# zhaodong-liu/GRAM

Hardware: AMD Instinct MI355X
Metric: users/sec @ beam=20 top-20 gen, Beauty T5-base; Recall@5 parity (higher is better)
Workload: dtype f16x3

## Files before the change

gram_amd/_lib.py:

```python
from __future__ import annotations

import ctypes as C
import os

_HERE = os.path.dirname(os.path.abspath(__file__))
LIB_PATH = os.environ.get("GRAM_LIB") or os.path.join(_HERE, "csrc", "libgram_hip.so")

GRAM_MAX_BEAMS = 64
GRAM_MAX_DEC_LEN = 64
GRAM_MAX_PASSAGE_LEN = 128
GRAM_MAX_LONG_PASSAGE_LEN = 512
GRAM_MAX_FUSED_LEN = 4096
GRAM_MAX_LONG_FUSED_LEN = 16384
GRAM_KEY_BITS_LONG_WORDS, GRAM_KEY_BITS_LONG_STRIDE = 512, 528
EPI_BF16, EPI_BF16_RELU, EPI_F32_ADD, EPI_F32, EPI_KV_BANK = range(5)
K_GEMM, K_ENC_ATTN, K_CROSS_ATTN, K_DEC_SELF_ATTN, K_ROWOPS, K_LSE, K_BEAM = range(7)
E_ARG, E_WORKSPACE, E_BEAM, E_NONFINITE = -1, -2, -3, -4
ABI_VERSION = 7
GRAM_TAIL_ENTRY_ROWS = 64
GRAM_TAIL_MAX_STEPS = 16
GRAM_MAX_USER_ITEMS = 4096
ITEMS_EXCLUDE, ITEMS_ALLOW = 0, 1
MAX_PIECES = 2
SPLIT_NPROD = (0, 1, 3)
# ... 136 lines not shown
    "gram_workspace_encoder_x_offset": (i64, [vp, C.c_int, C.c_int, C.c_int, C.c_int, C.c_int]),
    "gram_encode_fused": (C.c_int, [vp, vp, vp, C.c_int, C.c_int, C.c_int, vp, i64, C.c_int, C.c_int, vp, vp]),
    "gram_decode_step": (C.c_int, [vp, vp, vp, vp, C.c_int, C.c_int, C.c_int, C.c_int, C.c_int, C.c_int, vp, i64, vp, vp]),
    "gram_prof_pp_clock": (C.c_int, [C.POINTER(C.c_double), C.c_int]),
    "gram_prof_pp_clock_enable": (C.c_int, [C.c_int]),
    "gram_debug_set_gemm_variant": (C.c_int, [C.c_int]),
    "gram_gemm_stream_max_m": (C.c_int, []),
    "gram_debug_set_live_rows": (C.c_int, [C.c_int]),
    "gram_debug_set_token_tables": (C.c_int, [C.c_int]),
    "gram_debug_set_beam_chunked": (C.c_int, [C.c_int]),
    "gram_debug_set_beam_chunk_capacity": (C.c_int, [C.c_int]),
    "gram_debug_set_stage_pieces": (C.c_int, [C.POINTER(i32), C.c_int]),
    "gram_debug_stream_read": (C.c_int, [vp, C.c_size_t, vp, vp]),
    "gram_debug_stream_read_variant": (C.c_int, [vp, C.c_size_t, vp, C.c_int, C.c_int, vp]),
    "gram_prof_enable": (C.c_int, [C.c_uint32, C.c_int]),
    "gram_prof_reset": (C.c_int, []),
    "gram_prof_collect": (C.c_int, [C.c_int, C.POINTER(C.c_double), C.POINTER(i64), C.POINTER(C.c_double), C.POINTER(i64)]),
    "gram_rmsnorm_bf16_map": (C.c_int, [vp, vp, vp, C.c_int, C.c_int, f32, f32, vp, C.c_int, C.c_int, vp, vp]),
    "gram_generate_ex": (C.c_int, [vp, vp, vp, C.c_int, C.c_int, C.c_int, C.c_int, C.c_int, C.c_int, f32, C.POINTER(Trie),
                                   C.POINTER(Compaction), vp, i64, vp, vp, C.POINTER(i32), vp]),
    "gram_user_items_prepare": (C.c_int, [vp, C.c_int, vp, C.c_int, C.c_int, vp, vp, C.c_int, vp]),
    "gram_beam_step_sparse_items": (C.c_int, [C.POINTER(BeamState), C.POINTER(Trie), vp, vp, C.c_int, vp, C.c_int, C.c_int, C.c_int, vp,
                                              C.POINTER(UserItems), vp]),
    "gram_beam_step_sparse_split_items": (C.c_int, [C.POINTER(BeamState), C.POINTER(Trie), vp, vp, C.c_int, vp, C.c_int, C.c_int, C.c_int,
                                                    vp, C.c_int, C.POINTER(UserItems), vp]),
    "gram_greedy_step_items": (C.c_int, [C.POINTER(BeamState), C.POINTER(Trie), vp, C.c_int, C.c_int, C.POINTER(UserItems), vp]),
    "gram_generate_items": (C.c_int, [vp, vp, vp, C.c_int, C.c_int, C.c_int, C.c_int, C.c_int, C.c_int, f32, C.POINTER(Trie),
                                      C.POINTER(Compaction), C.POINTER(UserItems), vp, i64, vp, vp, C.POINTER(i32), vp]),
    "gram_encode_passages": (C.c_int, [vp, vp, vp, C.c_int, C.c_int, vp, i64, vp, vp]),
    "gram_gather_passage_x": (C.c_int, [vp, vp, vp, C.c_int, C.c_int, C.c_int, C.c_int, vp]),
    "gram_live_rows": (C.c_int, [C.POINTER(BeamState), C.POINTER(Trie), C.POINTER(LiveRows), vp]),
    "gram_dec_self_attn_live": (C.c_int, [vp, vp, vp, vp, vp, vp, C.c_int, C.c_int, vp, C.c_int, C.c_int, C.c_int, vp]),
    "gram_cross_attn_decode_live": (C.c_int, [vp, vp, vp, vp, vp, C.c_int, vp, vp, C.c_int, C.c_int, C.c_int, vp]),
    "gram_beam_step_sparse_live": (C.c_int, [C.POINTER(BeamState), C.POINTER(Trie), vp, vp, C.c_int, vp, C.c_int, C.c_int, vp, vp]),
    "gram_gemm_bf16_split": (C.c_int, [vp, vp, vp, C.c_int, C.c_int, C.c_int, C.c_int, C.c_int, C.c_int, C.POINTER(KVBank),
                                       C.POINTER(NormFusion), C.POINTER(Split), vp]),
    "gram_gemm_bf16_lse_split": (C.c_int, [vp, vp, vp, vp, C.c_int, C.c_int, C.c_int, C.c_int, C.c_int, C.POINTER(Split), vp]),
    "gram_embed_ex_split": (C.c_int, [vp, vp, C.c_int, vp, vp, vp, C.c_int, C.c_int, C.c_int, C.c_int, vp]),
    "gram_rmsnorm_bf16_split": (C.c_int, [vp, vp, vp, C.c_int, C.c_int, f32, f32, vp, C.c_int, C.c_int, vp, C.c_int, vp]),
    "gram_enc_self_attn_split": (C.c_int, [vp, vp, vp, vp, C.c_int, C.c_int, C.c_int, C.c_int, i64, vp]),
    "gram_cross_attn_decode_split": (C.c_int, [vp, vp, vp, vp, vp, C.c_int, C.c_int, C.c_int, C.c_int, vp, vp, C.c_int, i64, i64, vp, vp]),
    "gram_enc_self_attn_rows_split": (C.c_int, [vp, vp, vp, vp, vp, C.c_int, C.c_int, C.c_int, C.c_int, i64, vp]),
    "gram_enc_self_attn_long_split": (C.c_int, [vp, vp, vp, vp, C.c_int, C.c_int, C.c_int, C.c_int, i64, vp]),
    "gram_enc_self_attn_long_rows_split": (C.c_int, [vp, vp, vp, vp, vp, C.c_int, C.c_int, C.c_int, C.c_int, i64, vp]),
    "gram_model_set_max_passage_len": (C.c_int, [vp, C.c_int]),
    "gram_mask_key_bits": (C.c_int, [vp, vp, C.c_int, C.c_int, vp]),
    "gram_model_set_max_fused_len": (C.c_int, [vp, C.c_int]),
    "gram_mask_key_bits_long": (C.c_int, [vp, vp, C.c_int, C.c_int, vp]),
    "gram_cross_attn_long_scratch_bytes": (i64, [C.c_int, C.c_int, C.c_int]),
    "gram_cross_attn_long_split": (C.c_int, [vp, vp, vp, vp, vp, C.c_int, C.c_int, C.c_int, C.c_int, vp, vp, C.c_int, i64, i64, vp, vp, vp]),
    "gram_cross_attn_rows_long_split": (C.c_int, [vp, vp, vp, vp, vp, C.c_int, C.c_int, C.c_int, C.c_int, C.c_int, i64, i64, vp, vp, vp, vp]),
    "gram_dec_self_attn_split": (C.c_int, [vp, vp, vp, vp, vp, vp, C.c_int, C.c_int, vp, C.c_int, C.c_int, C.c_int, C.c_int, i64, i64, vp]),
    "gram_dec_self_attn_rows_split": (C.c_int, [vp, vp, vp, vp, vp, vp, vp, C.c_int, C.c_int, vp, C.c_int, C.c_int, C.c_int, C.c_int, i64, i64,
                                                vp]),
    "gram_beam_step_sparse_split": (C.c_int, [C.POINTER(BeamState), C.POINTER(Trie), vp, vp, C.c_int, vp, C.c_int, C.c_int, C.c_int,
                                              vp, C.c_int, vp]),
    "gram_generate": (C.c_int, [vp, vp, vp, C.c_int, C.c_int, C.c_int, C.c_int, C.c_int, C.c_int, f32, C.POINTER(Trie),
                                vp, i64, vp, vp, C.POINTER(i32), vp]),
    "gram_workspace_bytes_tf": (i64, [vp, C.c_int, C.c_int, C.c_int, C.c_int, C.c_int]),
    "gram_teacher_forced": (C.c_int, [vp, vp, vp, C.c_int, C.c_int, C.c_int, C.POINTER(Compaction), vp, vp, C.c_int, C.c_int, vp, i64,
                                      vp, vp, vp, vp]),
    "gram_dec_self_attn_tf_split": (C.c_int, [vp, vp, vp, C.c_int, C.c_int, C.c_int, C.c_int, i64, vp]),
    "gram_cross_attn_rows_split": (C.c_int, [vp, vp, vp, vp, vp, C.c_int, C.c_int, C.c_int, C.c_int, C.c_int, i64, i64, vp, vp, vp]),
    "gram_label_logprob_split": (C.c_int, [vp, vp, vp, C.c_int, vp, vp, C.c_int, C.c_int, C.c_int, C.c_int, vp, vp, vp]),
    "gram_cross_attn_probs_split": (C.c_int, [vp, vp, vp, vp, C.c_int, C.c_int, C.c_int, C.c_int, C.c_int, i64, i64, vp, vp]),
    "gram_xattn_head_sum": (C.c_int, [vp, vp, C.c_int, C.c_int, C.c_int, C.c_int, C.c_int, vp]),
    "gram_xattn_passage_scores": (C.c_int, [vp, vp, vp, C.c_int, C.c_int, C.c_int, C.c_int, f32, vp]),
    "gram_teacher_forced_ex": (C.c_int, [vp, vp, vp, C.c_int, C.c_int, C.c_int, C.POINTER(Compaction), vp, vp, C.c_int, C.c_int, vp, i64,
                                         vp, vp, vp, C.POINTER(XattnOut), vp]),
    "gram_cross_attn_token_scores_split": (C.c_int, [vp, vp, vp, C.c_int, C.c_int, C.c_int, C.c_int, C.c_int, i64, i64, vp, C.c_int, vp]),
    "gram_teacher_forced_scores": (C.c_int, [vp, vp, vp, C.c_int, C.c_int, C.c_int, C.POINTER(Compaction), vp, vp, C.c_int, C.c_int, vp,
                                             i64, vp, vp, vp, C.POINTER(XattnScores), vp]),
    "gram_dec_self_attn_tree_split": (C.c_int, [vp, vp, vp, vp, vp, C.c_int, C.c_int, C.c_int, C.c_int, C.c_int, i64, vp]),
    "gram_trie_repeat_tokens": (C.c_int, [vp, vp, C.c_int, C.c_int, vp]),
    "gram_trie_leaf_logprob_split": (C.c_int, [vp, vp, vp, C.c_int, vp, C.POINTER(TrieRows), C.c_int, C.c_int, C.c_int, vp, vp, vp, vp]),
    "gram_workspace_bytes_trie": (i64, [vp, C.c_int, C.c_int, C.c_int, C.c_int]),
    "gram_score_trie": (C.c_int, [vp, vp, vp, C.c_int, C.c_int, C.c_int, C.POINTER(Compaction), C.POINTER(Trie), C.POINTER(TrieRows), vp,
                                  i64, vp, vp, vp]),
    "gram_tail_forest": (C.c_int, [C.POINTER(BeamState), C.POINTER(Trie), C.POINTER(TrieTail), C.POINTER(Forest), C.c_int, vp]),
    "gram_tail_rowpos": (C.c_int, [C.POINTER(BeamState), C.POINTER(Trie), C.POINTER(Forest), vp]),
    "gram_scatter_rows": (C.c_int, [vp, vp, vp, C.c_int, C.c_int, C.c_int, vp]),
    "gram_cross_attn_entries_split": (C.c_int, [vp, vp, vp, vp, vp, C.c_int, C.c_int, C.c_int, C.c_int, vp, vp, C.c_int, i64, i64, vp,
                                                vp]),
    "gram_workspace_bytes_tail": (i64, [vp, C.c_int, C.c_int, C.c_int, C.c_int, C.c_int, C.c_int]),
    "gram_generate_tail": (C.c_int, [vp, vp, vp, C.c_int, C.c_int, C.c_int, C.c_int, C.c_int, C.c_int, f32, C.POINTER(Trie),
                                     C.POINTER(Compaction), C.POINTER(TrieTail), vp, i64, vp, vp, C.POINTER(i32), vp]),
    "gram_debug_set_tail_pass": (C.c_int, [C.c_int]),
    "gram_tail_pass_wanted": (C.c_int, [vp, C.c_int, C.c_int, C.c_int]),
    "gram_debug_set_tail_capacity": (C.c_int, [C.c_int]),
    "gram_debug_set_tail_level_capacity": (C.c_int, [C.c_int]),
    "gram_debug_tail_last": (C.c_int, [C.POINTER(i32)]),
    "gram_debug_workspace_beam_state": (C.c_int, [vp, vp, C.c_int, C.c_int, C.c_int, C.c_int, C.c_int, C.POINTER(BeamState)]),
    "gram_sample_step": (C.c_int, [C.POINTER(BeamState), C.POINTER(Trie), vp, vp, vp, C.c_int, vp, C.c_int, C.c_int, C.c_int, C.c_int,
                                   C.POINTER(SampleParams), vp, C.c_int, vp, vp, vp]),
    "gram_sample_step_items": (C.c_int, [C.POINTER(BeamState), C.POINTER(Trie), vp, vp, vp, C.c_int, vp, C.c_int, C.c_int, C.c_int, C.c_int,
                                         C.POINTER(SampleParams), vp, C.c_int, vp, vp, C.POINTER(UserItems), vp]),
    "gram_sample_finalize": (C.c_int, [C.POINTER(BeamState), C.c_int, vp, vp, vp, vp, vp, vp, vp]),
    "gram_sample_capacity": (C.c_int, []),
    "gram_debug_set_sample_capacity": (C.c_int, [C.c_int]),
    "gram_workspace_bytes_sample": (i64, [vp, C.c_int, C.c_int, C.c_int, C.c_int, C.c_int, C.c_int]),
    "gram_sample": (C.c_int, [vp, vp, vp, C.c_int, C.c_int, C.c_int, C.c_int, C.c_int, C.POINTER(Trie), C.POINTER(Compaction),
                              C.POINTER(SampleParams), vp, vp, i64, vp, vp, vp, C.POINTER(i32), vp]),
    "gram_sample_items": (C.c_int, [vp, vp, vp, C.c_int, C.c_int, C.c_int, C.c_int, C.c_int, C.POINTER(Trie), C.POINTER(Compaction),
                                    C.POINTER(UserItems), C.POINTER(SampleParams), vp, vp, i64, vp, vp, vp, C.POINTER(i32), vp]),
}

for _old, _new in (("gram_gemm_bf16", "gram_gemm_f16"), ("gram_gemm_bf16_ex", "gram_gemm_f16_ex"), ("gram_gemm_bf16_split", "gram_gemm_f16_split"),
                   ("gram_gemm_bf16_lse", "gram_gemm_f16_lse"), ("gram_gemm_bf16_lse_split", "gram_gemm_f16_lse_split"),
                   ("gram_rmsnorm_bf16", "gram_rmsnorm_f16"), ("gram_rmsnorm_bf16_map", "gram_rmsnorm_f16_map"),
                   ("gram_rmsnorm_bf16_split", "gram_rmsnorm_f16_split")):
    SIGNATURES[_new] = SIGNATURES[_old]

_lib = None


def load() -> C.CDLL:
    global _lib
    if _lib is not None:
        return _lib
    import torch
    if not os.path.exists(LIB_PATH):
        raise ImportError(
            f"{LIB_PATH} not found: the HIP extension is not built (run __graft_entry__.build() or "
            "`make -C gram_amd/csrc`).  gram_amd has no CPU fallback."
        )
    lib = C.CDLL(LIB_PATH)
    for name, (res, args) in SIGNATURES.items():
        fn = getattr(lib, name)
        fn.restype = res
        fn.argtypes = args
    if lib.gram_abi_version() != ABI_VERSION:
        raise ImportError("libgram_hip.so ABI version mismatch")
    _lib = lib
    return lib


class GramHipError(RuntimeError):
    pass


def piece_dtype():
    import torch
    return torch.float16 if load().gram_piece_format() == 1 else torch.bfloat16


def check(code: int, what: str) -> None:
    if code == 0:
        return
    names = {E_ARG: "GRAM_E_ARG (bad shape / unsupported size)", E_WORKSPACE: "GRAM_E_WORKSPACE",
             E_BEAM: "GRAM_E_BEAM (impossible beam state; HF would raise here)",
             E_NONFINITE: "GRAM_E_NONFINITE (a returned score is NaN / +inf: an activation left the range of the 16-bit pieces -- IEEE half, "
                          "|x| <= 65504; build and load the bfloat16 library: make -C gram_amd/csrc PIECE=bf16, GRAM_LIB=.../libgram_hip_bf16.so)"}
    raise GramHipError(f"{what} failed: {names.get(code, f'hipError {code}')}")
```

gram_amd/csrc/generate.hip:

```cpp
#include <stdlib.h>
#include <string.h>
#include <vector>

#include "common.h"
#include "prof.h"

struct gram_model {
  gram_model_desc_t d;
  std::vector<const float*> enc_ln1, enc_ln2, dec_ln1, dec_ln2, dec_ln3;
  std::vector<const void*> enc_wqkv, enc_wo, enc_wi, enc_wo2, dec_wqkv, dec_wo, dec_wq_x, dec_wo_x, dec_wi, dec_wo2;
  std::vector<float> s_enc_wqkv, s_enc_wo, s_enc_wi, s_enc_wo2, s_dec_wqkv, s_dec_wo, s_dec_wq_x, s_dec_wo_x, s_dec_wi, s_dec_wo2;
  float s_wkv = 1.f, s_lm = 1.f;
  const p16 *enc_qkv0 = nullptr, *dec_qkv0 = nullptr;
  int max_L = GRAM_MAX_PASSAGE_LEN;
  int max_S = GRAM_MAX_FUSED_LEN;
  bool long_xattn() const { return max_S > GRAM_MAX_FUSED_LEN; }
};

namespace {

struct Carve {
  char* base;
  int64_t off;
  explicit Carve(void* p) : base((char*)p), off(0) {}
// ... 367 lines not shown
template <typename SelfAttn, typename CrossAttn>
int decoder_layers(const gram_model* m, const Workspace& w, const int32_t* tokens, int n, bool qkv0_from_table, SelfAttn self_attn,
                   CrossAttn cross_attn, void* st) {
  const gram_model_desc_t& c = m->d;
  const int inner = c.n_heads * 64, F = c.d_ff;
  const Rows& r = w.dec;
  NormChain nc(m, w, r, n, st);
  TRY(nc.embed(tokens, 0, !qkv0_from_table));
  for (int i = 0; i < c.n_dec_layers; ++i) {
    TRY(sublayer(nc, {GRAM_STAGE_DEC_SELF, m->dec_ln1[i], m->dec_wqkv[i], m->s_dec_wqkv[i], r.qkv, C_PLANAR, r.ps_qkv, 3 * inner,
                      GRAM_EPI_BF16, r.attn, inner, m->dec_wo[i], m->s_dec_wo[i], i == 0 && qkv0_from_table},
                 i == 0, [&] { return self_attn(i); }));
    TRY(sublayer(nc, {GRAM_STAGE_DEC_CROSS, m->dec_ln2[i], m->dec_wq_x[i], m->s_dec_wq_x[i], r.qx, C_PLANAR, r.ps_qx, inner,
                      GRAM_EPI_BF16, r.attn, inner, m->dec_wo_x[i], m->s_dec_wo_x[i]},
                 false, [&] { return cross_attn(i); }));
    TRY(sublayer(nc, {GRAM_STAGE_DEC_FFN, m->dec_ln3[i], m->dec_wi[i], m->s_dec_wi[i], r.u, C_INTER, 0, F, GRAM_EPI_BF16_RELU, r.u, F,
                      m->dec_wo2[i], m->s_dec_wo2[i]},
                 false, no_mixer));
  }
  return 0;
}

int lm_head(const gram_model* m, const Workspace& w, int n, float* logits, float* lse_part, void* st) {
  const gram_model_desc_t& c = m->d;
  const int d = c.d_model, V = c.vocab;
  const float scale = c.tie_word_embeddings ? 1.0f / sqrtf((float)d) : 1.f;
  TRY(gram_rmsnorm_bf16_split(w.dec.x, c.dec_final_ln, w.dec.h, n, d, c.eps, scale, nullptr, 1, 1, nullptr, w.pieces, st));
  TRY(cap_inter(w, w.dec.h, n, d, GRAM_STAGE_LM_HEAD, st));
  const gram_split_t sp{w.pieces, 0, 0, 0, m->s_lm};
  if (lse_part) return gram_gemm_bf16_lse_split(w.dec.h, c.lm_head_bf16, logits, lse_part, n, V, d, w.pieces * d, V, &sp, st);
  return gram_gemm_bf16_split(w.dec.h, c.lm_head_bf16, logits, n, V, d, w.pieces * d, V, GRAM_EPI_F32, nullptr, nullptr, &sp, st);
}

int decode_step(const gram_model* m, const Workspace& w, const int32_t* tokens, const int32_t* anc, const uint8_t* mask, int B,
                int N, int L, int K, int R_cache, int Tmax, int t, float* logits, float* lse_part, const LiveStep* live,
                void* st) {
  const gram_model_desc_t& c = m->d;
  const int inner = c.n_heads * 64, H = c.n_heads;
  const int R = live ? live->n_rows : B * K, S = N * L;
  const size_t bank_layer = (size_t)B * H * S * 64;
  const size_t cache_layer = (size_t)Tmax * R_cache * inner;
  const Rows& r = w.dec;
  const p16* const table = token_table(m, m->dec_qkv0, GRAM_STAGE_DEC_SELF);
  TRY(decoder_layers(
      m, w, tokens, R, table != nullptr,
      [&](int i) {
        if (i == 0 && table)
          return gram_dec_self_attn_rows_split(table, tokens, w.kcache, w.vcache, anc, c.dec_bias_f32, r.attn, live ? R_cache : R, R,
                                               live ? live->rows : nullptr, H, t, Tmax, w.pieces, (int64_t)c.vocab * 3 * inner,
                                               w.ps_cache, st);
        return gram_dec_self_attn_split(r.qkv, w.kcache + i * cache_layer, w.vcache + i * cache_layer, anc, c.dec_bias_f32, r.attn,
                                        live ? R_cache : R, R, live ? live->rows : nullptr, H, t, Tmax, w.pieces, r.ps_qkv, w.ps_cache, st);
      },
      [&](int i) {
        if (m->long_xattn())
          return gram_cross_attn_long_split(r.qx, w.bank_k + i * bank_layer, w.bank_vt + i * bank_layer, mask, r.attn,
                                            live ? live->n_users : B, K, H, S, live ? live->users : nullptr,
                                            live ? live->rowpos : nullptr, w.pieces, r.ps_qx, w.ps_bank, w.key_bits, w.xa_scratch, st);
        return gram_cross_attn_decode_split(r.qx, w.bank_k + i * bank_layer, w.bank_vt + i * bank_layer, mask, r.attn,
                                            live ? live->n_users : B, K, H, S, live ? live->users : nullptr, live ? live->rowpos : nullptr,
                                            w.pieces, r.ps_qx, w.ps_bank, w.key_bits, st);
      },
      st));
  return lm_head(m, w, R, logits, lse_part, st);
}

int search_step(const gram_model* m, const Workspace& w, const gram_trie_t* trie, int cur_len, int rows_per_user, const int32_t* rowpos,
                const gram_user_items_t* items, void* st) {
  const gram_model_desc_t& c = m->d;
  if (items) {
    if (w.pieces > 1)
      return gram_beam_step_sparse_split_items(&w.beam, trie, w.dec.h, c.lm_head_f32, c.d_model, w.lse, c.vocab, cur_len, rows_per_user,
                                               rowpos, w.pieces, items, st);
    return gram_beam_step_sparse_items(&w.beam, trie, w.dec.h, c.lm_head_bf16, c.d_model, w.lse, c.vocab, cur_len, rows_per_user, rowpos,
                                       items, st);
  }
  if (w.pieces > 1)
    return gram_beam_step_sparse_split(&w.beam, trie, w.dec.h, c.lm_head_f32, c.d_model, w.lse, c.vocab, cur_len, rows_per_user, rowpos,
                                       w.pieces, st);
  if (rowpos) return gram_beam_step_sparse_live(&w.beam, trie, w.dec.h, c.lm_head_bf16, c.d_model, w.lse, c.vocab, cur_len, rowpos, st);
  return gram_beam_step_sparse(&w.beam, trie, w.dec.h, c.lm_head_bf16, c.d_model, w.lse, c.vocab, cur_len, rows_per_user, st);
}

int tail_pass(const gram_model* m, const Workspace& w, const uint8_t* mask, int B, int N, int L, int K, int Tmax, int t0, int n_rows,
              int n_entries, const int32_t* lvl_n, void* st) {
  const gram_model_desc_t& c = m->d;
  const int inner = c.n_heads * 64, H = c.n_heads, S = N * L, R = B * K;
  const size_t bank_layer = (size_t)B * H * S * 64;
  const size_t cache_layer = (size_t)Tmax * R * inner;
  const Rows& r = w.dec;
  const gram_forest_t& f = w.forest;
  const p16* const table = token_table(m, m->dec_qkv0, GRAM_STAGE_DEC_SELF);
  int nlev = f.n_levels, cut = 0;
  for (int g = 0; g < 2; ++g)
    for (int l = 0; l < f.n_levels; ++l)
      if (lvl_n[g * GRAM_TAIL_MAX_STEPS + l] > 0 && t0 + l >= Tmax - 1) cut = 1, nlev = l < nlev ? l : nlev;
  TRY(decoder_layers(
      m, w, f.tokens, n_rows, table != nullptr,
      [&](int i) {
        if (cut) {
          hipError_t e = hipMemsetAsync(r.attn, 0, (size_t)n_rows * inner * w.pieces * sizeof(p16), (hipStream_t)st);
          if (e != hipSuccess) return (int)e;
        }
        for (int g = 0; g < 2; ++g)
          for (int l = 0; l < nlev; ++l) {
            const int n = lvl_n[g * GRAM_TAIL_MAX_STEPS + l];
            if (n < 1) continue;
            const size_t tab = ((size_t)g * f.n_levels + l) * f.cap_rows;
            const int32_t* const rows_l = f.lvl_rows + tab;
            const int32_t* const anc_l = f.lvl_anc + ((size_t)g * f.n_levels + l) * Tmax * R;
            if (i == 0 && table)
              TRY(gram_dec_self_attn_rows_split(table, f.lvl_tokens + tab, w.kcache, w.vcache, anc_l, c.dec_bias_f32, r.qx, R, n, nullptr, H,
                                                t0 + l, Tmax, w.pieces, (int64_t)c.vocab * 3 * inner, w.ps_cache, st));
            else
              TRY(gram_dec_self_attn_rows_split(r.qkv, rows_l, w.kcache + i * cache_layer, w.vcache + i * cache_layer, anc_l, c.dec_bias_f32,
                                                r.qx, R, n, nullptr, H, t0 + l, Tmax, w.pieces, r.ps_qkv, w.ps_cache, st));
            TRY(gram_scatter_rows(r.qx, rows_l, r.attn, n, inner * w.pieces * (int)sizeof(p16), n_rows, st));
          }
        return 0;
      },
      [&](int i) {
        return gram_cross_attn_entries_split(r.qx, w.bank_k + i * bank_layer, w.bank_vt + i * bank_layer, mask, r.attn, n_entries, K, H, S,
                                             f.ent_users, f.ent_rows, w.pieces, r.ps_qx, w.ps_bank, w.key_bits, st);
      },
      st));
  TRY(lm_head(m, w, n_rows, nullptr, w.lse_part, st));
  return gram_lse_combine(w.lse_part, w.lse, n_rows, c.vocab / 64, st);
}
Workspace tail_view(const Workspace& w) {
  Workspace v = w;
  v.dec = w.tail;
  v.lse = w.tail_lse;
  v.lse_part = w.tail_lse_part;
  return v;
}

int g_tail_pass = -1;
int g_tail_cap = 0;
int g_tail_level_cap = 0;
int32_t g_tail_last[4] = {0, 0, 0, 0};
constexpr double kTailMinBankBytes = 256.0 * 1024 * 1024;
bool tail_wanted(const gram_model* m, int B, int N, int L) {
  if (g_tail_pass >= 0) return g_tail_pass != 0;
  const char* e = getenv("GRAM_TAIL_PASS");
  if (e && e[0] == '0') return false;
  if (e && e[0] == '1') return true;
  const int P = m->d.pieces > 1 ? m->d.pieces : 1;
  return 4.0 * B * m->d.n_heads * N * L * 64 * P >= kTailMinBankBytes;
}

}

extern "C" int gram_debug_set_tail_pass(int on) {
  g_tail_pass = on;
  return 0;
}
extern "C" int gram_tail_pass_wanted(const gram_model_t* m, int B, int N, int L) {
  if (!m || B < 1 || N < 1 || L < 1) return GRAM_E_ARG;
  return tail_wanted(m, B, N, L) ? 1 : 0;
}
extern "C" int gram_debug_set_tail_capacity(int rows) {
  g_tail_cap = rows < 0 ? 0 : rows;
  return 0;
}
extern "C" int gram_debug_workspace_beam_state(const gram_model_t* m, void* workspace, int B, int N, int L, int K, int max_length,
                                               gram_beam_state_t* out) {
  if (!workspace || !out || check_shapes(m, B, N, L, K, max_length)) return GRAM_E_ARG;
  *out = carve(m, workspace, B, N, L, K, max_length).beam;
  return 0;
}
extern "C" int gram_debug_set_tail_level_capacity(int rows) {
  g_tail_level_cap = rows < 0 ? 0 : rows;
  return 0;
}
extern "C" int gram_debug_tail_last(int32_t* out4) {
  if (!out4) return GRAM_E_ARG;
  memcpy(out4, g_tail_last, sizeof(g_tail_last));
  return 0;
}

extern "C" int gram_abi_version(void) { return GRAM_ABI_VERSION; }
extern "C" int gram_piece_format(void) { return GRAM_PIECE_FORMAT; }

extern "C" int gram_debug_set_stage_pieces(const int32_t* caps, int n) {
  if (caps && n != GRAM_STAGE_COUNT) return GRAM_E_ARG;
  for (int i = 0; i < GRAM_STAGE_COUNT; ++i) g_stage_cap[i] = caps ? (caps[i] < 1 ? 1 : caps[i]) : 99;
  return 0;
}

static int g_live_rows = -1;
extern "C" int gram_debug_set_live_rows(int on) {
  g_live_rows = on;
  return 0;
}
extern "C" int gram_debug_set_token_tables(int on) {
  g_token_tables = on;
  return 0;
}

extern "C" gram_model_t* gram_model_create(const gram_model_desc_t* d) {
  if (!d || d->vocab < 128 || d->d_model < 128 || d->d_ff < 128 || d->vocab % 128 || d->d_model % 128 || d->d_ff % 128 ||
      d->n_heads < 1 || d->n_heads > 16 ||
      (d->n_heads * 64) % 128 || d->d_model > 1024 || d->n_enc_layers < 1 || d->n_dec_layers < 1)
    return nullptr;
  if (d->pieces < 0 || d->pieces > GRAM_MAX_PIECES || (d->pieces > 1 && (!d->lm_head_f32 || !d->fold_norm))) return nullptr;
  gram_model* m = new gram_model();
  m->d = *d;
  auto own = [](auto& v, auto& p, int n) {
    v.assign(p, p + n);
    p = v.data();
  };
  gram_model_desc_t& c = m->d;
  own(m->enc_ln1, c.enc_ln1, c.n_enc_layers);
  own(m->enc_ln2, c.enc_ln2, c.n_enc_layers);
  own(m->enc_wqkv, c.enc_wqkv, c.n_enc_layers);
  own(m->enc_wo, c.enc_wo, c.n_enc_layers);
  own(m->enc_wi, c.enc_wi, c.n_enc_layers);
  own(m->enc_wo2, c.enc_wo2, c.n_enc_layers);
  own(m->dec_ln1, c.dec_ln1, c.n_dec_layers);
  own(m->dec_ln2, c.dec_ln2, c.n_dec_layers);
  own(m->dec_ln3, c.dec_ln3, c.n_dec_layers);
  own(m->dec_wqkv, c.dec_wqkv, c.n_dec_layers);
  own(m->dec_wo, c.dec_wo, c.n_dec_layers);
  own(m->dec_wq_x, c.dec_wq_x, c.n_dec_layers);
  own(m->dec_wo_x, c.dec_wo_x, c.n_dec_layers);
  own(m->dec_wi, c.dec_wi, c.n_dec_layers);
  own(m->dec_wo2, c.dec_wo2, c.n_dec_layers);
  {
    const float* ws = d->w_scales;
    auto take = [&](std::vector<float>& v, int n) {
      v.assign(n, 1.f);
      if (ws) {
        for (int i = 0; i < n; ++i) v[i] = 1.f / ws[i];
        ws += n;
      }
    };
    take(m->s_enc_wqkv, d->n_enc_layers);
// ... 577 lines not shown
```

include/gram_hip.h:

```cpp
#ifndef GRAM_HIP_H
#define GRAM_HIP_H

#include <stddef.h>
#include <stdint.h>

#ifdef __cplusplus
extern "C" {
#endif

#define GRAM_ABI_VERSION 7

#define GRAM_E_ARG (-1)
#define GRAM_E_WORKSPACE (-2)
#define GRAM_E_BEAM (-3)
#define GRAM_E_NONFINITE (-4)

#define GRAM_MAX_BEAMS 64
#define GRAM_MAX_DEC_LEN 64
#define GRAM_MAX_PASSAGE_LEN 128
#define GRAM_MAX_LONG_PASSAGE_LEN 512
#define GRAM_MAX_FUSED_LEN 4096
#define GRAM_MAX_LONG_FUSED_LEN 16384

enum gram_epilogue {
// ... 262 lines not shown
                  void* workspace, int64_t workspace_bytes, int64_t* sequences, float* scores,
                  int32_t* width_host, void* stream);

typedef struct {
  int32_t n_active;
  const int32_t* passage_map;
  const int64_t* ids;
  const uint8_t* mask;
  int32_t n_cached;
  int32_t cache_L;
  const float* cache_x;
  const int32_t* cache_slot;
} gram_compaction_t;
int gram_generate_ex(const gram_model_t* m, const int64_t* input_ids, const uint8_t* mask, int B, int N, int L,
                     int K, int nret, int max_length, float length_penalty, const gram_trie_t* trie_host,
                     const gram_compaction_t* compaction_host, void* workspace, int64_t workspace_bytes,
                     int64_t* sequences, float* scores, int32_t* width_host, void* stream);

int gram_generate_items(const gram_model_t* m, const int64_t* input_ids, const uint8_t* mask, int B, int N, int L, int K, int nret,
                        int max_length, float length_penalty, const gram_trie_t* trie_host, const gram_compaction_t* compaction_host,
                        const gram_user_items_t* items_host, void* workspace, int64_t workspace_bytes, int64_t* sequences,
                        float* scores, int32_t* width_host, void* stream);

struct gram_sample_params {
  float temperature;
  int32_t top_k;
  float top_p;
};
typedef struct gram_sample_params gram_sample_params_t;

int gram_sample_step(const gram_beam_state_t* st_host, const gram_trie_t* trie_host, const void* hidden_bf16, const void* lm_head_bf16,
                     const float* lm_head_f32, int d, const float* lse, int V, int cur_len, int rows_per_user, int pieces,
                     const gram_sample_params_t* params_host, const float* u, int u_stride, float* sample_logprob,
                     float* model_logprob, void* stream);
int gram_sample_step_items(const gram_beam_state_t* st_host, const gram_trie_t* trie_host, const void* hidden_bf16,
                           const void* lm_head_bf16, const float* lm_head_f32, int d, const float* lse, int V, int cur_len,
                           int rows_per_user, int pieces, const gram_sample_params_t* params_host, const float* u, int u_stride,
                           float* sample_logprob, float* model_logprob, const gram_user_items_t* items_host, void* stream);
int gram_sample_finalize(const gram_beam_state_t* st_host, int max_length, const float* model_logprob, const float* sample_logprob,
                         int64_t* sequences, float* seq_logprobs, float* sample_logprobs, int32_t* out_width, void* stream);
int gram_sample_capacity(void);
int gram_debug_set_sample_capacity(int candidates);

int64_t gram_workspace_bytes_sample(const gram_model_t* m, int B, int N, int L, int R, int max_length, int max_fanout);

int gram_sample(const gram_model_t* m, const int64_t* input_ids, const uint8_t* mask, int B, int N, int L, int R, int max_length,
                const gram_trie_t* trie_host, const gram_compaction_t* compaction_host, const gram_sample_params_t* params_host,
                const float* uniforms, void* workspace, int64_t workspace_bytes, int64_t* sequences, float* seq_logprobs,
                float* sample_logprobs, int32_t* width_host, void* stream);
int gram_sample_items(const gram_model_t* m, const int64_t* input_ids, const uint8_t* mask, int B, int N, int L, int R, int max_length,
                      const gram_trie_t* trie_host, const gram_compaction_t* compaction_host, const gram_user_items_t* items_host,
                      const gram_sample_params_t* params_host, const float* uniforms, void* workspace, int64_t workspace_bytes,
                      int64_t* sequences, float* seq_logprobs, float* sample_logprobs, int32_t* width_host, void* stream);

#define GRAM_TAIL_MAX_STEPS 16
#define GRAM_TAIL_ENTRY_ROWS 64
typedef struct {
  const int32_t* sub_rows;
  int32_t d_tail;
  int32_t steps;
} gram_trie_tail_t;
typedef struct {
  int32_t* tokens;
  int32_t* pos;
  int32_t* parent;
  int32_t* root;
  int32_t* node;
  int32_t* user_off;
  int32_t* ent_off;
  int32_t* ent_users;
  int32_t* ent_rows;
  int32_t* rowpos;
  int32_t* counts;
  int32_t* slot;
  int32_t* lvl_rows;
  int32_t* lvl_tokens;
  int32_t* lvl_anc;
  int32_t cap_rows, cap_entries, n_levels, pad_;
} gram_forest_t;
int gram_tail_forest(const gram_beam_state_t* st_host, const gram_trie_t* trie_host, const gram_trie_tail_t* tail_host,
                     const gram_forest_t* forest_host, int t, void* stream);
int gram_tail_rowpos(const gram_beam_state_t* st_host, const gram_trie_t* trie_host, const gram_forest_t* forest_host, void* stream);
int gram_scatter_rows(const void* src, const int32_t* rows, void* dst, int n, int row_bytes, int dst_rows, void* stream);
int gram_cross_attn_entries_split(const void* q, const void* k_layer, const void* vt_layer, const uint8_t* mask, void* out,
                                  int n_entries, int K, int H, int S, const int32_t* ent_users, const int32_t* ent_rows, int pieces,
                                  int64_t q_pstride, int64_t bank_pstride, const uint32_t* key_bits, void* stream);
int64_t gram_workspace_bytes_tail(const gram_model_t* m, int B, int N, int L, int K, int max_length, int steps);
int gram_generate_tail(const gram_model_t* m, const int64_t* input_ids, const uint8_t* mask, int B, int N, int L, int K, int nret,
                       int max_length, float length_penalty, const gram_trie_t* trie_host, const gram_compaction_t* compaction_host,
                       const gram_trie_tail_t* tail_host, void* workspace, int64_t workspace_bytes, int64_t* sequences,
                       float* scores, int32_t* width_host, void* stream);

int gram_encode_passages(const gram_model_t* m, const int64_t* ids, const uint8_t* mask, int P, int L,
                         void* workspace, int64_t workspace_bytes, float* x_out, void* stream);
int64_t gram_workspace_encoder_x_offset(const gram_model_t* m, int B, int N, int L, int K, int max_length);
int gram_gather_passage_x(const float* cache_x, const int32_t* slot, float* x, int n, int L, int cache_L, int d,
                          void* stream);


int64_t gram_workspace_bytes_tf(const gram_model_t* m, int B, int N, int L, int C, int T);

int gram_teacher_forced(const gram_model_t* m, const int64_t* input_ids, const uint8_t* mask, int B, int N, int L,
                        const gram_compaction_t* compaction_host, const int32_t* dec_ids, const int32_t* labels, int C, int T,
                        void* workspace, int64_t workspace_bytes, float* logits, float* token_logp, float* seq_logp, void* stream);

int gram_dec_self_attn_tf_split(const void* qkv, const float* bias, void* out, int n_seq, int T, int H, int pieces,
                                int64_t qkv_pstride, void* stream);

int gram_cross_attn_rows_split(const void* q, const void* k_layer, const void* vt_layer, const uint8_t* mask, void* out, int B, int Q,
                               int H, int S, int pieces, int64_t q_pstride, int64_t bank_pstride, const uint32_t* key_bits,
                               int32_t* rowmap, void* stream);
int gram_cross_attn_rows_long_split(const void* q, const void* k_layer, const void* vt_layer, const uint8_t* mask, void* out, int B,
                                    int Q, int H, int S, int pieces, int64_t q_pstride, int64_t bank_pstride, const uint32_t* key_bits,
                                    float* scratch, int32_t* rowmap, void* stream);

int gram_label_logprob_split(const void* hidden, const void* lm_head_bf16, const float* lm_head_f32, int d, const float* lse,
                             const int32_t* labels, int n_seq, int T, int V, int pieces, float* token_logp, float* seq_logp,
                             void* stream);


int gram_cross_attn_probs_split(const void* q, const void* k_layer, const uint8_t* mask, float* probs, int B, int Q, int H, int S,
                                int pieces, int64_t q_pstride, int64_t bank_pstride, const uint32_t* key_bits, void* stream);

int gram_xattn_head_sum(const float* probs, float* acc, int B, int Q, int H, int S, int first, void* stream);

int gram_xattn_passage_scores(const float* acc, const uint8_t* mask, float* scores, int B, int Q, int N, int L, float denom,
                              void* stream);

typedef struct {
  float* probs;
  float* layer_probs;
  float* token_scores;
  float* passage_scores;
} gram_xattn_out_t;

int gram_teacher_forced_ex(const gram_model_t* m, const int64_t* input_ids, const uint8_t* mask, int B, int N, int L,
                           const gram_compaction_t* compaction_host, const int32_t* dec_ids, const int32_t* labels, int C, int T,
                           void* workspace, int64_t workspace_bytes, float* logits, float* token_logp, float* seq_logp,
                           const gram_xattn_out_t* attn_host, void* stream);

int gram_cross_attn_token_scores_split(const void* q, const void* k_layer, float* acc, int B, int Q, int H, int S, int pieces,
                                       int64_t q_pstride, int64_t bank_pstride, const uint32_t* key_bits, int first, void* stream);

typedef struct {
  float* token_scores;
  float* passage_scores;
} gram_xattn_scores_t;

int gram_teacher_forced_scores(const gram_model_t* m, const int64_t* input_ids, const uint8_t* mask, int B, int N, int L,
                               const gram_compaction_t* compaction_host, const int32_t* dec_ids, const int32_t* labels, int C, int T,
                               void* workspace, int64_t workspace_bytes, float* logits, float* token_logp, float* seq_logp,
                               const gram_xattn_scores_t* scores_host, void* stream);


typedef struct {
  const int32_t* tokens;
  const int32_t* pos;
  const int32_t* anc;
  const int32_t* row_node;
  const int32_t* node_row;
  const int32_t* node_tok;
  const int32_t* node_leaf;
  int32_t Q, Tq;
  int32_t n_nodes, n_leaves;
} gram_trie_rows_t;

int gram_dec_self_attn_tree_split(const void* qkv, const int32_t* pos, const int32_t* anc, const float* bias, void* out, int B, int Q,
                                  int Tq, int H, int pieces, int64_t qkv_pstride, void* stream);

int gram_trie_repeat_tokens(const int32_t* tokens, int32_t* out, int B, int Q, void* stream);

int gram_trie_leaf_logprob_split(const void* hidden, const void* lm_head_bf16, const float* lm_head_f32, int d, const float* lse,
                                 const gram_trie_rows_t* rows_host, int B, int V, int pieces, float* row_edge, float* leaf_logp,
                                 float* node_logp, void* stream);

int64_t gram_workspace_bytes_trie(const gram_model_t* m, int B, int N, int L, int Q);

int gram_score_trie(const gram_model_t* m, const int64_t* input_ids, const uint8_t* mask, int B, int N, int L,
                    const gram_compaction_t* compaction_host, const gram_trie_t* trie_host, const gram_trie_rows_t* rows_host,
                    void* workspace, int64_t workspace_bytes, float* leaf_logp, float* node_logp, void* stream);

enum gram_kernel_kind {
  GRAM_K_GEMM = 0,
  GRAM_K_ENC_ATTN = 1,
  GRAM_K_CROSS_ATTN = 2,
  GRAM_K_DEC_SELF_ATTN = 3,
  GRAM_K_ROWOPS = 4,
  GRAM_K_LSE = 5,
  GRAM_K_BEAM = 6,
  GRAM_K_COUNT = 7
};
int gram_prof_enable(uint32_t kind_mask, int max_events);
int gram_prof_reset(void);
int gram_prof_collect(int kind, double* total_ms, int64_t* launches, double* work, int64_t* dropped);

int gram_prof_pp_clock_enable(int on);
int gram_prof_pp_clock(double* ghz, int reset);

int gram_debug_set_gemm_variant(int variant);

int gram_debug_stream_read(const void* src, size_t bytes, void* sink, void* stream);
int gram_debug_stream_read_variant(const void* src, size_t bytes, void* sink, int variant, int wgs, void* stream);

int gram_debug_set_live_rows(int on);
int gram_debug_set_token_tables(int on);
int gram_debug_set_tail_pass(int on);
int gram_tail_pass_wanted(const gram_model_t* m, int B, int N, int L);
int gram_debug_set_tail_capacity(int rows);
int gram_debug_set_tail_level_capacity(int rows);
int gram_debug_tail_last(int32_t* out4);
int gram_debug_workspace_beam_state(const gram_model_t* m, void* workspace, int B, int N, int L, int K, int max_length,
                                    gram_beam_state_t* out);
int gram_debug_set_beam_chunked(int mode);
int gram_debug_set_beam_chunk_capacity(int candidates);
enum gram_stage {
  GRAM_STAGE_ENC_ATTN = 0,
  GRAM_STAGE_ENC_FFN = 1,
  GRAM_STAGE_BANK_K = 2,
  GRAM_STAGE_BANK_V = 3,
  GRAM_STAGE_DEC_SELF = 4,
  GRAM_STAGE_DEC_CROSS = 5,
  GRAM_STAGE_DEC_FFN = 6,
  GRAM_STAGE_LM_HEAD = 7,
  GRAM_STAGE_COUNT = 8
};
int gram_debug_set_stage_pieces(const int32_t* caps, int n);

int gram_gemm_f16(const void* A, const void* W, void* C, int M, int N, int K, int lda, int ldc, int epilogue,
                  const gram_kv_bank_t* bank_host, void* stream);
int gram_gemm_f16_ex(const void* A, const void* W, void* C, int M, int N, int K, int lda, int ldc, int epilogue,
                     const gram_kv_bank_t* bank_host, const gram_norm_fusion_t* nf_host, void* stream);
int gram_gemm_f16_split(const void* A, const void* W, void* C, int M, int N, int kc, int lda, int ldc, int epilogue,
                        const gram_kv_bank_t* bank_host, const gram_norm_fusion_t* nf_host, const gram_split_t* split_host, void* stream);
int gram_gemm_f16_lse(const void* A, const void* W, float* logits, float* lse_part, int M, int N, int K, int lda, int ldc, void* stream);
int gram_gemm_f16_lse_split(const void* A, const void* W, float* logits, float* lse_part, int M, int N, int kc, int lda, int ldc,
                            const gram_split_t* split_host, void* stream);
int gram_rmsnorm_f16(const float* x, const float* w, void* out_f16, int rows, int d, float eps, float scale, const float* pos, int N,
                     int L, void* stream);
int gram_rmsnorm_f16_map(const float* x, const float* w, void* out_f16, int rows, int d, float eps, float scale, const float* pos,
                         int N, int L, const int32_t* passage_map, void* stream);
int gram_rmsnorm_f16_split(const float* x, const float* w, void* out_f16, int rows, int d, float eps, float scale, const float* pos,
                           int N, int L, const int32_t* passage_map, int pieces, void* stream);

int gram_abi_version(void);
int gram_piece_format(void);

#ifdef __cplusplus
}
#endif
#endif
```

Baseline: 3237.

## Add single-launch forest self-attention kernel for tail pass decoder layers

Result: faster. 3276 (median of 6 runs) (+1.2%).

```diff
diff --git a/gram_amd/_lib.py b/gram_amd/_lib.py
--- a/gram_amd/_lib.py
+++ b/gram_amd/_lib.py
@@ -242,6 +242,9 @@
     "gram_scatter_rows": (C.c_int, [vp, vp, vp, C.c_int, C.c_int, C.c_int, vp]),
     "gram_cross_attn_entries_split": (C.c_int, [vp, vp, vp, vp, vp, C.c_int, C.c_int, C.c_int, C.c_int, vp, vp, C.c_int, i64, i64, vp,
                                                 vp]),
+    "gram_dec_self_attn_forest_split": (C.c_int, [vp, vp, vp, vp, vp, vp, vp, vp, vp, vp, C.c_int, C.c_int, C.c_int, C.c_int, C.c_int,
+                                                  C.c_int, C.c_int, i64, i64, vp]),
+    "gram_debug_set_tail_forest_attn": (C.c_int, [C.c_int]),
     "gram_workspace_bytes_tail": (i64, [vp, C.c_int, C.c_int, C.c_int, C.c_int, C.c_int, C.c_int]),
     "gram_generate_tail": (C.c_int, [vp, vp, vp, C.c_int, C.c_int, C.c_int, C.c_int, C.c_int, C.c_int, f32, C.POINTER(Trie),
                                      C.POINTER(Compaction), C.POINTER(TrieTail), vp, i64, vp, vp, C.POINTER(i32), vp]),
diff --git a/gram_amd/csrc/forest_attn.hip b/gram_amd/csrc/forest_attn.hip
--- /dev/null
+++ b/gram_amd/csrc/forest_attn.hip
@@ -0,0 +1,156 @@
+#include <stdlib.h>
+
+#include "common.h"
+#include "prof.h"
+#include "self_attn_row.h"
+
+namespace {
+
+__device__ __forceinline__ int clampi(int v, int lo, int hi) { return v < lo ? lo : (v > hi ? hi : v); }
+
+template <int S>
+__global__ __launch_bounds__(256) void dec_self_attn_forest_kernel(
+    const p16* __restrict__ qkv, const int32_t* __restrict__ qkv_rows, const p16* __restrict__ kcache, const p16* __restrict__ vcache,
+    const int32_t* __restrict__ anc, const int32_t* __restrict__ pos, const int32_t* __restrict__ parent,
+    const int32_t* __restrict__ root, const float* __restrict__ bias, p16* __restrict__ out, int n_rows, int R, int H, int t0, int Tmax,
+    int nlev, long qkv_ps, long cache_ps, int xcd_chunk) {
+  constexpr int U = 2, ML = GRAM_TAIL_MAX_STEPS;
+  static_assert(ML % U == 0, "the in-pass ancestors are taken in whole batches");
+  const int w = blockIdx.x, tid = threadIdx.x;
+  const int i = xcd_chunk > 0 ? (w & 7) * xcd_chunk + (w >> 3) : w;
+  if (i >= n_rows) return;
+  const int p = pos[i], l = p - t0;
+  if (l < 0 || l >= nlev || p >= Tmax) return;
+  const int inner = H * 64, h = tid >> 4;
+  const int rt = clampi(root[i], 0, R - 1);
+  auto src = [&](int r) { return qkv + (size_t)(qkv_rows ? qkv_rows[r] : r) * 3 * inner + 4 * tid; };
+  const float* const bias_h = bias + h * GRAM_MAX_DEC_LEN;
+
+  const p16* const row = src(i);
+  p16x4 q4[S], k4[S], v4[S];
+#pragma unroll
+  for (int pc = 0; pc < S; ++pc) {
+    q4[pc] = *reinterpret_cast<const p16x4*>(row + pc * qkv_ps);
+    k4[pc] = *reinterpret_cast<const p16x4*>(row + pc * qkv_ps + inner);
+    v4[pc] = *reinterpret_cast<const p16x4*>(row + pc * qkv_ps + 2 * inner);
+  }
+  auto cache_issue = [&](int j0, p16x4(&kk)[U][S], p16x4(&vv)[U][S]) {
+    int a[U];
+#pragma unroll
+    for (int u = 0; u < U; ++u) a[u] = anc[(size_t)min(j0 + u, t0 - 1) * R + rt];
+#pragma unroll
+    for (int u = 0; u < U; ++u) {
+      const size_t off = ((size_t)min(j0 + u, t0 - 1) * R + clampi(a[u], 0, R - 1)) * inner + 4 * tid;
+#pragma unroll
+      for (int pc = 0; pc < S; ++pc) {
+        kk[u][pc] = *reinterpret_cast<const p16x4*>(kcache + pc * cache_ps + off);
+        vv[u][pc] = *reinterpret_cast<const p16x4*>(vcache + pc * cache_ps + off);
+      }
+    }
+  };
+  auto pass_issue = [&](int e0, const int(&rows)[U], p16x4(&kk)[U][S], p16x4(&vv)[U][S]) {
+    const p16* ar[U];
+#pragma unroll
+    for (int u = 0; u < U; ++u) ar[u] = src(rows[u]);
+#pragma unroll
+    for (int u = 0; u < U; ++u) {
+      if (e0 + u < l) {
+#pragma unroll
+        for (int pc = 0; pc < S; ++pc) {
+          kk[u][pc] = *reinterpret_cast<const p16x4*>(ar[u] + pc * qkv_ps + inner);
+          vv[u][pc] = *reinterpret_cast<const p16x4*>(ar[u] + pc * qkv_ps + 2 * inner);
+        }
+      }
+    }
+  };
+
+  float qf[4], m = -INFINITY, lsum = 0.f, acc[4] = {0.f, 0.f, 0.f, 0.f};
+  auto eat = [&](int j0, int end, const p16x4(&kk)[U][S], const p16x4(&vv)[U][S]) {
+#pragma unroll
+    for (int u = 0; u < U; ++u) {
+      if (j0 + u < end) {
+        float kj[4], vj[4];
+        sa_sum<S>(kk[u], kj);
+        sa_sum<S>(vv[u], vj);
+        sa_step(qf, kj, vj, bias_h[p - (j0 + u)], m, lsum, acc);
+      }
+    }
+  };
+
+  p16x4 ck[U][S], cv[U][S];
+  if (t0 > 0) cache_issue(0, ck, cv);
+  int asc[ML];
+#pragma unroll
+  for (int e = 0; e < ML; ++e) asc[e] = i;
+  {
+    int cur = i;
+#pragma unroll
+    for (int e = ML - 1; e >= 0; --e) {
+      if (e < l) {
+        cur = clampi(parent[cur], 0, n_rows - 1);
+        asc[e] = cur;
+      }
+    }
+  }
+  p16x4 pk[U][S], pv[U][S];
+  {
+    int rows[U];
+#pragma unroll
+    for (int u = 0; u < U; ++u) rows[u] = asc[u];
+    if (l > 0) pass_issue(0, rows, pk, pv);
+  }
+
+  sa_sum<S>(q4, qf);
+  if (t0 > 0) eat(0, t0, ck, cv);
+  for (int j0 = U; j0 < t0; j0 += U) {
+    cache_issue(j0, ck, cv);
+    eat(j0, t0, ck, cv);
+  }
+  if (l > 0) eat(t0, p, pk, pv);
+#pragma unroll
+  for (int e0 = U; e0 < ML; e0 += U) {
+    if (e0 < l) {
+      int rows[U];
+#pragma unroll
+      for (int u = 0; u < U; ++u) rows[u] = asc[e0 + u];
+      pass_issue(e0, rows, pk, pv);
+      eat(t0 + e0, p, pk, pv);
+    }
+  }
+  float kn[4], vn[4];
+  sa_sum<S>(k4, kn);
+  sa_sum<S>(v4, vn);
+  sa_step(qf, kn, vn, bias_h[0], m, lsum, acc);
+  sa_store<S>(out + (size_t)i * inner * S, 4 * tid, lsum, acc);
+}
+
+}
+
+extern "C" int gram_dec_self_attn_forest_split(const void* qkv, const int32_t* qkv_rows, const void* kcache, const void* vcache,
+                                               const int32_t* anc, const int32_t* pos, const int32_t* parent, const int32_t* root,
+                                               const float* bias, void* out, int n_rows, int R, int H, int t0, int Tmax, int nlev,
+                                               int pieces, int64_t qkv_pstride, int64_t cache_pstride, void* stream) {
+  if (!qkv || !kcache || !vcache || !anc || !pos || !parent || !root || !bias || !out || n_rows < 1 || n_rows > INT32_MAX / 4 ||
+      R < 1 || H < 1 || H > 16 || t0 < 0 || t0 >= Tmax || Tmax > GRAM_MAX_DEC_LEN || nlev < 1 || nlev > GRAM_TAIL_MAX_STEPS ||
+      pieces < 1 || pieces > GRAM_MAX_PIECES)
+    return GRAM_E_ARG;
+  if (pieces > 1 && (qkv_pstride < 1 || cache_pstride < (int64_t)Tmax * R * H * 64)) return GRAM_E_ARG;
+  hipStream_t st = (hipStream_t)stream;
+  gram_prof::Scope prof(GRAM_K_DEC_SELF_ATTN, st, 2.0 * 4 * n_rows * H * 64 * pieces);
+  static const bool by_xcd = [] {
+    const char* e = getenv("GRAM_FOREST_ROW_ORDER");
+    return !(e && e[0] == '0');
+  }();
+  const int chunk = by_xcd ? (n_rows + 7) / 8 : 0;
+  const dim3 grid(by_xcd ? 8 * chunk : n_rows), block(H * 16);
+  if (pieces == 2)
+    hipLaunchKernelGGL(dec_self_attn_forest_kernel<2>, grid, block, 0, st, (const p16*)qkv, qkv_rows, (const p16*)kcache,
+                       (const p16*)vcache, anc, pos, parent, root, bias, (p16*)out, n_rows, R, H, t0, Tmax, nlev, (long)qkv_pstride,
+                       (long)cache_pstride, chunk);
+  else
+    hipLaunchKernelGGL(dec_self_attn_forest_kernel<1>, grid, block, 0, st, (const p16*)qkv, qkv_rows, (const p16*)kcache,
+                       (const p16*)vcache, anc, pos, parent, root, bias, (p16*)out, n_rows, R, H, t0, Tmax, nlev, (long)qkv_pstride,
+                       (long)cache_pstride, chunk);
+  GRAM_CHECK_LAUNCH();
+  return 0;
+}
diff --git a/gram_amd/csrc/generate.hip b/gram_amd/csrc/generate.hip
--- a/gram_amd/csrc/generate.hip
+++ b/gram_amd/csrc/generate.hip
@@ -473,6 +473,16 @@
   return gram_beam_step_sparse(&w.beam, trie, w.dec.h, c.lm_head_bf16, c.d_model, w.lse, c.vocab, cur_len, rows_per_user, st);
 }
 
+int g_tail_forest_attn = -1;
+constexpr int kForestAttnMinRows = 16384;
+bool tail_forest_attn_wanted(int n_rows) {
+  if (g_tail_forest_attn >= 0) return g_tail_forest_attn != 0;
+  const char* e = getenv("GRAM_TAIL_FOREST_ATTN");
+  if (e && e[0] == '0') return false;
+  if (e && e[0] == '1') return true;
+  return n_rows >= kForestAttnMinRows;
+}
+
 int tail_pass(const gram_model* m, const Workspace& w, const uint8_t* mask, int B, int N, int L, int K, int Tmax, int t0, int n_rows,
               int n_entries, const int32_t* lvl_n, void* st) {
   const gram_model_desc_t& c = m->d;
@@ -486,12 +496,22 @@
   for (int g = 0; g < 2; ++g)
     for (int l = 0; l < f.n_levels; ++l)
       if (lvl_n[g * GRAM_TAIL_MAX_STEPS + l] > 0 && t0 + l >= Tmax - 1) cut = 1, nlev = l < nlev ? l : nlev;
+  const bool forest_attn = tail_forest_attn_wanted(n_rows);
   TRY(decoder_layers(
       m, w, f.tokens, n_rows, table != nullptr,
       [&](int i) {
         if (cut) {
           hipError_t e = hipMemsetAsync(r.attn, 0, (size_t)n_rows * inner * w.pieces * sizeof(p16), (hipStream_t)st);
           if (e != hipSuccess) return (int)e;
+        }
+        if (forest_attn) {
+          if (i == 0 && table)
+            return gram_dec_self_attn_forest_split(table, f.tokens, w.kcache, w.vcache, w.beam.anc, f.pos, f.parent, f.root, c.dec_bias_f32,
+                                                   r.attn, n_rows, R, H, t0, Tmax, nlev, w.pieces, (int64_t)c.vocab * 3 * inner, w.ps_cache,
+                                                   st);
+          return gram_dec_self_attn_forest_split(r.qkv, nullptr, w.kcache + i * cache_layer, w.vcache + i * cache_layer, w.beam.anc, f.pos,
+                                                 f.parent, f.root, c.dec_bias_f32, r.attn, n_rows, R, H, t0, Tmax, nlev, w.pieces, r.ps_qkv,
+                                                 w.ps_cache, st);
         }
         for (int g = 0; g < 2; ++g)
           for (int l = 0; l < nlev; ++l) {
@@ -544,6 +564,10 @@
 
 extern "C" int gram_debug_set_tail_pass(int on) {
   g_tail_pass = on;
+  return 0;
+}
+extern "C" int gram_debug_set_tail_forest_attn(int on) {
+  g_tail_forest_attn = on;
   return 0;
 }
 extern "C" int gram_tail_pass_wanted(const gram_model_t* m, int B, int N, int L) {
diff --git a/include/gram_hip.h b/include/gram_hip.h
--- a/include/gram_hip.h
+++ b/include/gram_hip.h
@@ -368,6 +368,10 @@
                      const gram_forest_t* forest_host, int t, void* stream);
 int gram_tail_rowpos(const gram_beam_state_t* st_host, const gram_trie_t* trie_host, const gram_forest_t* forest_host, void* stream);
 int gram_scatter_rows(const void* src, const int32_t* rows, void* dst, int n, int row_bytes, int dst_rows, void* stream);
+int gram_dec_self_attn_forest_split(const void* qkv, const int32_t* qkv_rows, const void* kcache, const void* vcache, const int32_t* anc,
+                                    const int32_t* pos, const int32_t* parent, const int32_t* root, const float* bias, void* out,
+                                    int n_rows, int R, int H, int t0, int Tmax, int nlev, int pieces, int64_t qkv_pstride,
+                                    int64_t cache_pstride, void* stream);
 int gram_cross_attn_entries_split(const void* q, const void* k_layer, const void* vt_layer, const uint8_t* mask, void* out,
                                   int n_entries, int K, int H, int S, const int32_t* ent_users, const int32_t* ent_rows, int pieces,
                                   int64_t q_pstride, int64_t bank_pstride, const uint32_t* key_bits, void* stream);
@@ -491,6 +495,7 @@
 int gram_debug_set_live_rows(int on);
 int gram_debug_set_token_tables(int on);
 int gram_debug_set_tail_pass(int on);
+int gram_debug_set_tail_forest_attn(int on);
 int gram_tail_pass_wanted(const gram_model_t* m, int B, int N, int L);
 int gram_debug_set_tail_capacity(int rows);
 int gram_debug_set_tail_level_capacity(int rows);
```
